# shanice-l/UNOPose

Hardware: AMD Instinct MI355X
Metric: (query,ref) pairs/sec forward (higher is better)
Workload: dtype bf16; 1 GPU; UNOPose.forward, batch 32 pairs/GPU, 2048 query pts, 5000->2048 reference pts, 196 coarse pts, 518x518 crops, DINOv2 ViT-B/14 reg4, random-init (trained-like) weights

## Files before the change

### include/unopose_hip.h

```cpp
#ifndef UNOPOSE_HIP_H
#define UNOPOSE_HIP_H

#include <stdint.h>

#ifdef __cplusplus
extern "C" {
#endif

#define UNOPOSE_OK 0
#define UNOPOSE_EINVAL 1
#define UNOPOSE_ELAUNCH 2
#define UNOPOSE_ENOMEM 3

typedef void *unopose_stream_t;

int unopose_abi_version(void);
const char *unopose_last_error(void);


int unopose_furthest_point_sampling(const float *xyz, int B, int N, int M,
                                    int32_t *idx, unopose_stream_t stream);

int unopose_gather_points(const float *points, const int32_t *idx, int B, int C,
                          int N, int M, float *out, unopose_stream_t stream);
// ... 41 lines not shown
                                const float *w, int M, int N, float thresh,
                                float eps, float *R, float *t,
                                unopose_stream_t stream);

int unopose_pe_image_bytes(void);
int unopose_pe_pack_weights(const float *w1, const float *b1, const float *w2, const float *b2,
                            const float *w3, const float *b3, void *image, unopose_stream_t stream);
int unopose_pe_group_mlp_max_packed(const float *xyz, int B, int N, float radius, int nsample,
                                    const void *image, float *out, unopose_stream_t stream);

int unopose_pe_group_mlp_max_packed_cand(const float *xyz, int B, int N, float radius, int nsample,
                                         const void *image, const int *cand_in, const int *cand_cnt_in,
                                         int cand_stride, int *cand_out, int *cand_cnt_out, float *out,
                                         unopose_stream_t stream);
int unopose_pe_group_mlp_max_packed_out(const float *xyz, int B, int N, float radius, int nsample, const void *image,
                                        const int *cand_in, const int *cand_cnt_in, int cand_stride, int *cand_out,
                                        int *cand_cnt_out, void *out, int out_ld, int out_split, unopose_stream_t stream);

int unopose_geo_embedding(const float *points, int B, int n, const void *wd_hi,
                          const void *wd_lo, const void *wa_hi, const void *wa_lo,
                          const float *bias_sum, const float *div_term,
                          float sigma_d, float factor_a, int reduce_mean, int split,
                          int out_bf16, int32_t *knn_ws, void *out,
                          unopose_stream_t stream);

int unopose_geo_embedding_table(const float *points, int B, int n, const float *tab_d, int rows_d, const float *tab_a, int rows_a,
                                const float *bias_sum, const float *w_d, const float *div_term, int hinv, int npoint, float sigma_d,
                                float factor_a, int reduce_mean, int out_bf16, int32_t *knn_ws, void *out,
                                unopose_stream_t stream);

// ... 197 lines not shown
```

### unopose_amd/_lib.py

```python
import ctypes
import os

import torch

_HERE = os.path.dirname(os.path.abspath(__file__))
SO_PATH = os.environ.get("UNOPOSE_LIB") or os.path.join(_HERE, "libunopose_hip.so")

_lib = None

_P = ctypes.c_void_p
_I = ctypes.c_int
_F = ctypes.c_float
_L = ctypes.c_long

SIGNATURES = {
    "unopose_furthest_point_sampling": [_P, _I, _I, _I, _P, _P],
    "unopose_gather_points": [_P, _P, _I, _I, _I, _I, _P, _P],
    "unopose_gather_points_grad": [_P, _P, _I, _I, _I, _I, _P, _P],
    "unopose_ball_query": [_P, _P, _I, _I, _I, _F, _I, _P, _P],
    "unopose_group_points": [_P, _P, _I, _I, _I, _I, _I, _P, _P],
    "unopose_group_points_grad": [_P, _P, _I, _I, _I, _I, _I, _P, _P],
    "unopose_three_nn": [_P, _P, _I, _I, _I, _P, _P, _P],
    "unopose_three_interpolate": [_P, _P, _P, _I, _I, _I, _I, _P, _P],
    "unopose_three_interpolate_grad": [_P, _P, _P, _I, _I, _I, _I, _P, _P],
# ... 66 lines not shown
    "unopose_overlap_scores": [_P, _I, _I, _I, _I, _I, _P, _P],
    "unopose_copy_rows": [_P, _L, _P, _L, _I, _I, _P],
    "unopose_nan_to_num_multi": [_P, _P, _I, _L, _F, _F, _F, _P],
    "unopose_rigid_rows_bf16": [_P, _I, _I, _P, _P, _P, _P],
    "unopose_token_sum_bf16": [_P, _I, _I, _I, _P, _P],
    "unopose_pose_score": [_P, _P, _I, _I, _F, _P, _P],
    "unopose_render_depth": [_P, _I, _P, _I, _P, _P, _I, _I, _I, _P, _P],
    "unopose_bmm_f32": [_P, ctypes.c_long, ctypes.c_long, ctypes.c_long, ctypes.c_long, _P, ctypes.c_long, ctypes.c_long, ctypes.c_long, ctypes.c_long, _P, _I, _I, _I, _I, _I, _F, _P],
    "unopose_split_bf16x2": [_P, ctypes.c_long, _I, _P, _P],
    "unopose_linear_f32x3": [_P, _P, _P, _P, _P, ctypes.c_long, _I, _I, _I, _P],
    "unopose_pe_image_bytes": [],
    "unopose_pe_pack_weights": [_P, _P, _P, _P, _P, _P, _P, _P],
    "unopose_pe_group_mlp_max_packed": [_P, _I, _I, _F, _I, _P, _P, _P],
    "unopose_pe_group_mlp_max_packed_cand": [_P, _I, _I, _F, _I, _P, _P, _P, _I, _P, _P, _P, _P],
    "unopose_pe_group_mlp_max_packed_out": [_P, _I, _I, _F, _I, _P, _P, _P, _I, _P, _P, _P, _I, _I, _P],
    "unopose_linear_f32x3_bf16": [_P, _P, _P, _P, _P, ctypes.c_long, _I, _I, _P],
    "unopose_pe_group_mlp_max": [_P, _I, _I, _F, _I, _P, _P, _P, _P, _P, _P, _I, _P, _P],
    "unopose_geo_embedding": [_P, _I, _I, _P, _P, _P, _P, _P, _P, _F, _F, _I, _I, _I, _P, _P, _P],
    "unopose_geo_embedding_train_workgroups": [_I, _I],
    "unopose_geo_embedding_train_forward": [_P, _I, _I, _P, _I, _P, _I, _P, _P, _P, _I, _F, _F, _I, _P, _P, _P, _P],
    "unopose_geo_embedding_train_backward": [_P, _P, _I, _I, _I, _I, _I, _F, _F, _I, _P, _P, _P, _P, _P, _P],
    "unopose_geo_embedding_table": [_P, _I, _I, _P, _I, _P, _I, _P, _P, _P, _I, _I, _F, _F, _I, _I, _P, _P, _P],
}


def lib():
    global _lib
    if _lib is None:
        if not os.path.exists(SO_PATH):
            raise RuntimeError(
# ... 70 lines not shown
```

### unopose_amd/csrc/pe.hip

```cpp
#include "common.h"
#include "jacobi3.h"

namespace unopose {

constexpr int PE_SCAN_STEPS = 4;

__device__ __forceinline__ int cd_row(int r, int h) { return (r & 3) + 8 * (r >> 2) + 4 * h; }

constexpr int PE_GDIM = 8, PE_GCELLS = PE_GDIM * PE_GDIM * PE_GDIM;
struct PeGrid {
  float ox, oy, oz, ihx, ihy, ihz;
  int nx, ny, nz;
  const u16 *start;
  const u16 *order;
  uint32_t *bits;
};
__device__ __forceinline__ int pe_cell(float v, float o, float ih, int n) { return max(0, min(n - 1, (int)((v - o) * ih))); }

template <typename NT>
__device__ __forceinline__ int pe_centre_frame(const float *sx, const float *sy, const float *sz, int N, int S,
                                               float radius, float r2, int lane, float cx, float cy, float cz,
                                               NT *nbr, Vec3 &xp, Vec3 &yp, Vec3 &zp, const int *cand = nullptr,
                                               int ncand = -1, const PeGrid *grid = nullptr) {
  int cnt = 0, first = 0;
// ... 279 lines not shown
    L->w2l[o][pe_kperm(c)] = f2bf(v - bf2f(h));
  }
  for (int e = tid; e < 128 * 64; e += 256) {
    const int o = e >> 6, c = e & 63;
    const float v = w3[e];
    const u16 h = f2bf(v);
    const int kp = pe_kperm(c) ^ ((o & 7) << 3);
    L->w3h[o][kp] = h;
    L->w3l[o][kp] = f2bf(v - bf2f(h));
  }
  if (tid < 32) L->b1[tid] = b1[tid];
  if (tid < 64) L->b2[tid] = b2[tid];
  if (tid < 128) L->b3[tid] = b3[tid];
}

constexpr int PE_NW = 4;
__global__ __launch_bounds__(PE_NW * 64, 8 / PE_NW) void pe_group_mlp_max_bf16x3_kernel(
    const float *__restrict__ xyz, int N, float radius, int S, int cpw, const uint4 *__restrict__ image,
    const int *__restrict__ cand_in, const int *__restrict__ cand_cnt_in, int cand_stride, int *__restrict__ cand_out,
    int *__restrict__ cand_cnt_out, float *__restrict__ out, int out_ld, int out_split, int use_grid) {
  extern __shared__ float4 smem4[];
  PeLdsB *L = reinterpret_cast<PeLdsB *>(smem4);
  float *sx = reinterpret_cast<float *>(L + 1);
  float *sy = sx + N, *sz = sy + N;
  float *stage_all = sz + N;
  u16 *nbr_all = reinterpret_cast<u16 *>(stage_all + PE_NW * 128);
  u16 *gstart = nbr_all + PE_NW * S;
  u16 *gorder = gstart + PE_GCELLS + 2;
  const int b = blockIdx.y, tid = threadIdx.x, lane = tid & 63, wave = tid >> 6;
  const int half = lane >> 5, col = lane & 31;
  u16 *nbr = nbr_all + wave * S;
  float *stage = stage_all + wave * 128;
  const float *P = xyz + (size_t)b * N * 3;

  for (int e = tid; e < N * 3; e += PE_NW * 64) {
    const float v = P[e];
    const int p = e / 3, comp = e - p * 3;
    (comp == 0 ? sx : comp == 1 ? sy : sz)[p] = v;
  }
  for (int e = tid; e < (int)(sizeof(PeLdsB) / 16); e += PE_NW * 64) smem4[e] = *reinterpret_cast<const float4 *>(image + e);
  __syncthreads();
  const float r2 = radius * radius;
  PeGrid grid;
  if (use_grid) {
    static_assert(PE_NW * 128 >= PE_GCELLS, "the cell counters borrow the staging area");
    uint32_t *cnt32 = reinterpret_cast<uint32_t *>(stage_all);
    float *red = reinterpret_cast<float *>(nbr_all);
    float lo[3] = {3e38f, 3e38f, 3e38f}, hi[3] = {-3e38f, -3e38f, -3e38f};
    for (int p = tid; p < N; p += PE_NW * 64) {
      lo[0] = fminf(lo[0], sx[p]), hi[0] = fmaxf(hi[0], sx[p]);
      lo[1] = fminf(lo[1], sy[p]), hi[1] = fmaxf(hi[1], sy[p]);
      lo[2] = fminf(lo[2], sz[p]), hi[2] = fmaxf(hi[2], sz[p]);
    }
#pragma unroll
    for (int a = 0; a < 3; ++a) {
      lo[a] = -wave_max_f32(-lo[a]);
      hi[a] = wave_max_f32(hi[a]);
      if (lane == 0) red[wave * 6 + a] = lo[a], red[wave * 6 + 3 + a] = hi[a];
    }
    for (int c = tid; c < PE_GCELLS; c += PE_NW * 64) cnt32[c] = 0u;
    __syncthreads();
    float org[3], ih[3];
    int nd[3];
#pragma unroll
    for (int a = 0; a < 3; ++a) {
      float l = red[a], h = red[3 + a];
      for (int w = 1; w < PE_NW; ++w) l = fminf(l, red[w * 6 + a]), h = fmaxf(h, red[w * 6 + 3 + a]);
      const float ext = h - l, h0 = radius * 1.001f;
      int n = (int)(ext / h0) + 1;
      float edge = h0;
      if (!(n <= PE_GDIM)) n = PE_GDIM, edge = fmaxf(h0, ext / (float)PE_GDIM * 1.001f);
      org[a] = __int_as_float(__builtin_amdgcn_readfirstlane(__float_as_int(l)));
      ih[a] = __int_as_float(__builtin_amdgcn_readfirstlane(__float_as_int(1.f / edge)));
      nd[a] = __builtin_amdgcn_readfirstlane(max(n, 1));
    }
    grid.ox = org[0], grid.oy = org[1], grid.oz = org[2], grid.ihx = ih[0], grid.ihy = ih[1], grid.ihz = ih[2];
    grid.nx = nd[0], grid.ny = nd[1], grid.nz = nd[2];
    grid.start = gstart, grid.order = gorder, grid.bits = reinterpret_cast<uint32_t *>(stage);
    auto cell_of = [&](int p) {
      return (pe_cell(sz[p], grid.oz, grid.ihz, grid.nz) * grid.ny + pe_cell(sy[p], grid.oy, grid.ihy, grid.ny)) * grid.nx +
             pe_cell(sx[p], grid.ox, grid.ihx, grid.nx);
    };
    for (int p = tid; p < N; p += PE_NW * 64) atomicAdd(&cnt32[cell_of(p)], 1u);
    __syncthreads();
    {
      constexpr int CPT = PE_GCELLS / (PE_NW * 64);
      static_assert(CPT * PE_NW * 64 == PE_GCELLS, "cells divide among the threads");
      uint32_t c[CPT], sum = 0;
#pragma unroll
      for (int e = 0; e < CPT; ++e) c[e] = cnt32[tid * CPT + e], sum += c[e];
      uint32_t incl = sum;
#pragma unroll
      for (int d = 1; d < 64; d <<= 1) {
        const uint32_t t = __shfl_up(incl, d);
        if (lane >= d) incl += t;
      }
      uint32_t *wtot = reinterpret_cast<uint32_t *>(red) + 32;
      if (lane == 63) wtot[wave] = incl;
      __syncthreads();
      uint32_t base = incl - sum;
      for (int w = 0; w < wave; ++w) base += wtot[w];
#pragma unroll
      for (int e = 0; e < CPT; ++e) {
        gstart[tid * CPT + e] = (u16)base;
        cnt32[tid * CPT + e] = base;
        base += c[e];
      }
      if (tid == PE_NW * 64 - 1) gstart[PE_GCELLS] = (u16)base;
    }
    __syncthreads();
    for (int p = tid; p < N; p += PE_NW * 64) gorder[atomicAdd(&cnt32[cell_of(p)], 1u)] = (u16)p;
    __syncthreads();
  }

  for (int ci = 0; ci < cpw; ++ci) {
    const int j = (blockIdx.x * PE_NW + wave) * cpw + ci;
    if (j >= N) break;
    const float cx = sx[j], cy = sy[j], cz = sz[j];
    Vec3 xp, yp, zp;
    const int *cand = nullptr;
    int ncand = -1;
    if (cand_in) {
      ncand = cand_cnt_in[(size_t)b * N + j];
      cand = cand_in + ((size_t)b * N + j) * cand_stride;
    }
    const int cnt = pe_centre_frame(sx, sy, sz, N, S, radius, r2, lane, cx, cy, cz, nbr, xp, yp, zp, cand, ncand, use_grid ? &grid : nullptr);
    if (cand_out) {
      int *co = cand_out + ((size_t)b * N + j) * S;
      for (int l = lane; l < S; l += 64) co[l] = nbr[l];
      if (lane == 0) cand_cnt_out[(size_t)b * N + j] = cnt <= S ? cnt : -1;
    }

    f32x16 rmax[4];
#pragma unroll
    for (int t = 0; t < 4; ++t)
#pragma unroll
      for (int r = 0; r < 16; ++r) rmax[t][r] = 0.f;
    const int S_eff = min(S, (max(min(cnt, S), 1) + 31) & ~31);
    for (int t0 = 0; t0 < S_eff; t0 += 32) {
      asm volatile("" ::: "memory");
      const int k = nbr[t0 + col];
      const float dx = sx[k] - cx, dy = sy[k] - cy, dz = sz[k] - cz;
      const Vec3 q = v3(dx / radius, dy / radius, dz / radius);
      float f[8] = {dx, dy, dz, dot(xp, q), dot(yp, q), dot(zp, q), 0.f, 0.f};
      if (half) {
#pragma unroll
        for (int e = 0; e < 8; ++e) f[e] = 0.f;
      }
      const bf16x8_hl x = split8_bf16(f);
      struct Grp {
        bf16x8_hl w[4];
        float4 b[4];
      } ga, gb;
      auto load_l1 = [&](Grp &g) {
        g.w[0].hi = *reinterpret_cast<const bf16x8 *>(&L->w1h[col][half * 8]);
        g.w[0].lo = *reinterpret_cast<const bf16x8 *>(&L->w1l[col][half * 8]);
#pragma unroll
        for (int q = 0; q < 4; ++q) g.b[q] = *reinterpret_cast<const float4 *>(&L->b1[8 * q + 4 * half]);
      };
      auto load_l2 = [&](Grp &g, int ot) {
#pragma unroll
        for (int ks = 0; ks < 2; ++ks) {
          g.w[ks].hi = *reinterpret_cast<const bf16x8 *>(&L->w2h[ot * 32 + col][ks * 16 + half * 8]);
          g.w[ks].lo = *reinterpret_cast<const bf16x8 *>(&L->w2l[ot * 32 + col][ks * 16 + half * 8]);
        }
#pragma unroll
        for (int q = 0; q < 4; ++q) g.b[q] = *reinterpret_cast<const float4 *>(&L->b2[ot * 32 + 8 * q + 4 * half]);
      };
      auto load_l3 = [&](Grp &g, int ot) {
        const int row = ot * 32 + col;
#pragma unroll
        for (int ks = 0; ks < 4; ++ks) {
          const int kp = (ks * 16 + half * 8) ^ ((row & 7) << 3);
          g.w[ks].hi = *reinterpret_cast<const bf16x8 *>(&L->w3h[row][kp]);
          g.w[ks].lo = *reinterpret_cast<const bf16x8 *>(&L->w3l[row][kp]);
        }
#pragma unroll
        for (int q = 0; q < 4; ++q) g.b[q] = *reinterpret_cast<const float4 *>(&L->b3[ot * 32 + 8 * q + 4 * half]);
      };
      auto init = [&](f32x16 &h, const Grp &g) {
#pragma unroll
        for (int q = 0; q < 4; ++q) {
          h[4 * q + 0] = g.b[q].x;
          h[4 * q + 1] = g.b[q].y;
          h[4 * q + 2] = g.b[q].z;
          h[4 * q + 3] = g.b[q].w;
        }
      };
      bf16x8_hl a1[2], a2[4];
      auto relu_split = [&](const f32x16 &h, bf16x8_hl *o) {
#pragma unroll
        for (int s2 = 0; s2 < 2; ++s2) {
          float v[8];
#pragma unroll
          for (int e = 0; e < 8; ++e) v[e] = fmaxf(h[s2 * 8 + e], 0.f);
          o[s2] = split8_bf16(v);
        }
      };
      load_l1(ga);
      load_l2(gb, 0);
      __builtin_amdgcn_sched_barrier(0);
      {
        f32x16 h1;
        init(h1, ga);
        h1 = mfma3_hh_hl_lh_32x32(ga.w[0], x, h1);
        load_l2(ga, 1);
        __builtin_amdgcn_sched_barrier(0);
        relu_split(h1, a1);
      }
      {
        f32x16 h2;
        init(h2, gb);
#pragma unroll
        for (int ks = 0; ks < 2; ++ks) h2 = mfma3_hh_hl_lh_32x32(gb.w[ks], a1[ks], h2);
        load_l3(gb, 0);
        __builtin_amdgcn_sched_barrier(0);
        relu_split(h2, a2);
        init(h2, ga);
#pragma unroll
        for (int ks = 0; ks < 2; ++ks) h2 = mfma3_hh_hl_lh_32x32(ga.w[ks], a1[ks], h2);
        load_l3(ga, 1);
        __builtin_amdgcn_sched_barrier(0);
        relu_split(h2, a2 + 2);
      }
#pragma unroll
      for (int ot = 0; ot < 4; ++ot) {
        Grp &g = (ot & 1) ? ga : gb;
        f32x16 h3;
        init(h3, g);
#pragma unroll
        for (int ks = 0; ks < 4; ++ks) h3 = mfma3_hh_hl_lh_32x32(g.w[ks], a2[ks], h3);
        if (ot + 2 < 4) {
          load_l3(g, ot + 2);
          __builtin_amdgcn_sched_barrier(0);
        }
#pragma unroll
        for (int r = 0; r < 16; ++r) rmax[ot][r] = fmaxf(rmax[ot][r], h3[r]);
      }
    }
#pragma unroll
    for (int t = 0; t < 4; ++t)
#pragma unroll
      for (int r = 0; r < 16; ++r) {
        float v = rmax[t][r];
        v = fmaxf(v, dpp_f32<0x111, 0xF>(v, 0.f));
        v = fmaxf(v, dpp_f32<0x112, 0xF>(v, 0.f));
        v = fmaxf(v, dpp_f32<0x114, 0xF>(v, 0.f));
        v = fmaxf(v, dpp_f32<0x118, 0xF>(v, 0.f));
        v = fmaxf(v, dpp_f32<0x142, 0xA>(v, 0.f));
        if (col == 31) stage[t * 32 + cd_row(r, half)] = v;
      }
    __builtin_amdgcn_fence(__ATOMIC_RELEASE, "wavefront");
    __builtin_amdgcn_wave_barrier();
    __builtin_amdgcn_fence(__ATOMIC_ACQUIRE, "wavefront");
    float *O = out + ((size_t)b * N + j) * out_ld;
    if (!out_split) {
      O[lane] = stage[lane];
      O[lane + 64] = stage[lane + 64];
    } else {
      uint32_t *O32 = reinterpret_cast<uint32_t *>(O);
#pragma unroll
      for (int q = 0; q < 2; ++q) {
        const int d = lane + 64 * q, blk = d >> 5, w = d & 31, k = blk * 32 + (w & 15) * 2;
        const float v0 = stage[k], v1 = stage[k + 1];
        const uint32_t h = cvt_pk_bf16_f32(v0, v1);
        O32[d] = (w & 16) ? cvt_pk_bf16_lo(v0, v1, h) : h;
      }
    }
    __builtin_amdgcn_wave_barrier();
  }
}

}

using namespace unopose;

extern "C" {

int unopose_pe_image_bytes(void) { return (int)sizeof(PeLdsB); }

int unopose_pe_pack_weights(const float *w1, const float *b1, const float *w2, const float *b2, const float *w3,
                            const float *b3, void *image, unopose_stream_t stream) {
  UNOPOSE_REQUIRE(w1 && b1 && w2 && b2 && w3 && b3 && image, "pe_pack_weights: null pointer");
  hipLaunchKernelGGL(pe_pack_weights_kernel, dim3(1), dim3(256), 0, (hipStream_t)stream, w1, b1, w2, b2, w3, b3,
// ... 2 lines not shown
}

int unopose_pe_group_mlp_max_packed(const float *xyz, int B, int N, float radius, int nsample, const void *image,
                                    float *out, unopose_stream_t stream) {
  return unopose_pe_group_mlp_max_packed_cand(xyz, B, N, radius, nsample, image, nullptr, nullptr, 0, nullptr, nullptr,
                                              out, stream);
}

int unopose_pe_group_mlp_max_packed_cand(const float *xyz, int B, int N, float radius, int nsample, const void *image,
                                         const int *cand_in, const int *cand_cnt_in, int cand_stride, int *cand_out,
                                         int *cand_cnt_out, float *out, unopose_stream_t stream) {
  return unopose_pe_group_mlp_max_packed_out(xyz, B, N, radius, nsample, image, cand_in, cand_cnt_in, cand_stride, cand_out,
                                             cand_cnt_out, out, 128, 0, stream);
}

int unopose_pe_group_mlp_max_packed_out(const float *xyz, int B, int N, float radius, int nsample, const void *image,
                                        const int *cand_in, const int *cand_cnt_in, int cand_stride, int *cand_out,
                                        int *cand_cnt_out, void *out, int out_ld, int out_split, unopose_stream_t stream) {
  UNOPOSE_REQUIRE(xyz && image && out, "pe_group_mlp_max_packed: null pointer");
  UNOPOSE_REQUIRE(out_ld >= 128 && (out_split == 0 || out_split == 1), "pe_group_mlp_max_packed: bad output stride / mode");
  UNOPOSE_REQUIRE((cand_in == nullptr) == (cand_cnt_in == nullptr) && (cand_out == nullptr) == (cand_cnt_out == nullptr) &&
                      (!cand_in || cand_stride >= 1),
                  "pe_group_mlp_max_packed: candidate list and its counts go together");
  UNOPOSE_REQUIRE(B >= 0 && N >= 1 && nsample >= 32 && nsample % 32 == 0 && B <= 65535,
                  "pe_group_mlp_max_packed: nsample must be a positive multiple of 32 (got %d)", nsample);
  if (B == 0) return UNOPOSE_OK;
  size_t lds = sizeof(PeLdsB) + ((size_t)3 * N + PE_NW * 128) * 4 + (size_t)PE_NW * nsample * 2;
  UNOPOSE_REQUIRE(N < 65536 && lds <= 160 * 1024, "pe_group_mlp_max_packed: N=%d nsample=%d exceed the LDS tile", N, nsample);
  const size_t grid_bytes = ((size_t)PE_GCELLS + 2 + (size_t)N) * 2;
  const int use_grid = radius > 0.f && N <= 4096 && N >= 256 && lds + grid_bytes <= 160 * 1024 && (lds + grid_bytes <= 80 * 1024 || lds > 80 * 1024);
  if (use_grid) lds += grid_bytes;
  lds = (lds + 15) & ~(size_t)15;
  static bool opt[64];
  if (lds_optin(opt, (const void *)pe_group_mlp_max_bf16x3_kernel, 160 * 1024, "pe_group_mlp_max_packed") != UNOPOSE_OK) return UNOPOSE_ELAUNCH;
  const long centres = (long)B * N;
  const int cpw = centres >= 65536 ? 16 : centres >= 32768 ? 8 : centres >= 8192 ? 4 : centres >= 2048 ? 2 : 1;
  dim3 grid(cdiv(N, PE_NW * cpw), B);
  hipLaunchKernelGGL(pe_group_mlp_max_bf16x3_kernel, grid, dim3(PE_NW * 64), lds, (hipStream_t)stream, xyz, N, radius, nsample,
                     cpw, (const uint4 *)image, cand_in, cand_cnt_in, cand_stride, cand_out, cand_cnt_out, (float *)out, out_ld, out_split, use_grid);
  return check_launch("pe_group_mlp_max_packed");
}

int unopose_pe_group_mlp_max(const float *xyz, int B, int N, float radius, int nsample, const float *w1,
                             const float *b1, const float *w2, const float *b2, const float *w3, const float *b3,
                             int bf16x3, float *out, unopose_stream_t stream) {
  UNOPOSE_REQUIRE(xyz && w1 && b1 && w2 && b2 && w3 && b3 && out, "pe_group_mlp_max: null pointer");
  UNOPOSE_REQUIRE(B >= 0 && N >= 1 && nsample >= 32 && nsample % 32 == 0 && B <= 65535,
                  "pe_group_mlp_max: nsample must be a positive multiple of 32 (got %d)", nsample);
  if (B == 0) return UNOPOSE_OK;
  const size_t lds = sizeof(PeLds) + ((size_t)3 * N + 4 * (size_t)nsample + 4 * 128) * 4;
  UNOPOSE_REQUIRE(lds <= 160 * 1024, "pe_group_mlp_max: N=%d nsample=%d exceed the LDS tile", N, nsample);
  static bool opt[64];
  if (lds_optin(opt, (const void *)pe_group_mlp_max_kernel, 160 * 1024, "pe_group_mlp_max") != UNOPOSE_OK) return UNOPOSE_ELAUNCH;
  const long centres = (long)B * N;
  const int cpw = centres >= 32768 ? 8 : centres >= 8192 ? 4 : centres >= 2048 ? 2 : 1;
// ... 10 lines not shown
```

Measured before the change: 1099 pairs/s.

## Split PE kernel into producer/consumer waves with LDS ring buffer

Restructures the point-embedding group+MLP+max kernel so four producer waves do the neighbour search and local frame while four consumer waves run the MFMA MLP. The two sides hand work through an LDS ring of neighbour lists and frames, using ticket counters and ready/freed flags. The point is to overlap the scalar-heavy ball query with the matrix-core MLP. Work per workgroup is now sized so the launch has about 512 workgroups. The old kernel is kept as a reference entry point, and the spin-wait sync adds deadlock and occupancy risk.

```diff
diff --git a/include/unopose_hip.h b/include/unopose_hip.h
--- a/include/unopose_hip.h
+++ b/include/unopose_hip.h
@@ -79,6 +79,9 @@
                                          int cand_stride, int *cand_out, int *cand_cnt_out, float *out,
                                          unopose_stream_t stream);
 int unopose_pe_group_mlp_max_packed_out(const float *xyz, int B, int N, float radius, int nsample, const void *image,
+                                        const int *cand_in, const int *cand_cnt_in, int cand_stride, int *cand_out,
+                                        int *cand_cnt_out, void *out, int out_ld, int out_split, unopose_stream_t stream);
+int unopose_pe_group_mlp_max_packed_ref(const float *xyz, int B, int N, float radius, int nsample, const void *image,
                                         const int *cand_in, const int *cand_cnt_in, int cand_stride, int *cand_out,
                                         int *cand_cnt_out, void *out, int out_ld, int out_split, unopose_stream_t stream);
 
diff --git a/unopose_amd/_lib.py b/unopose_amd/_lib.py
--- a/unopose_amd/_lib.py
+++ b/unopose_amd/_lib.py
@@ -104,6 +104,7 @@
     "unopose_pe_group_mlp_max_packed": [_P, _I, _I, _F, _I, _P, _P, _P],
     "unopose_pe_group_mlp_max_packed_cand": [_P, _I, _I, _F, _I, _P, _P, _P, _I, _P, _P, _P, _P],
     "unopose_pe_group_mlp_max_packed_out": [_P, _I, _I, _F, _I, _P, _P, _P, _I, _P, _P, _P, _I, _I, _P],
+    "unopose_pe_group_mlp_max_packed_ref": [_P, _I, _I, _F, _I, _P, _P, _P, _I, _P, _P, _P, _I, _I, _P],
     "unopose_linear_f32x3_bf16": [_P, _P, _P, _P, _P, ctypes.c_long, _I, _I, _P],
     "unopose_pe_group_mlp_max": [_P, _I, _I, _F, _I, _P, _P, _P, _P, _P, _P, _I, _P, _P],
     "unopose_geo_embedding": [_P, _I, _I, _P, _P, _P, _P, _P, _P, _F, _F, _I, _I, _I, _P, _P, _P],
diff --git a/unopose_amd/csrc/pe.hip b/unopose_amd/csrc/pe.hip
--- a/unopose_amd/csrc/pe.hip
+++ b/unopose_amd/csrc/pe.hip
@@ -317,9 +317,315 @@
   if (tid < 128) L->b3[tid] = b3[tid];
 }
 
-constexpr int PE_NW = 4;
-__global__ __launch_bounds__(PE_NW * 64, 8 / PE_NW) void pe_group_mlp_max_bf16x3_kernel(
+template <int NW>
+__device__ PeGrid pe_build_grid(const float *sx, const float *sy, const float *sz, int N, float radius, int tid, int lane, int wave,
+                                uint32_t *cnt32, float *red, u16 *gstart, u16 *gorder) {
+  PeGrid grid;
+  float lo[3] = {3e38f, 3e38f, 3e38f}, hi[3] = {-3e38f, -3e38f, -3e38f};
+  for (int p = tid; p < N; p += NW * 64) {
+    lo[0] = fminf(lo[0], sx[p]), hi[0] = fmaxf(hi[0], sx[p]);
+    lo[1] = fminf(lo[1], sy[p]), hi[1] = fmaxf(hi[1], sy[p]);
+    lo[2] = fminf(lo[2], sz[p]), hi[2] = fmaxf(hi[2], sz[p]);
+  }
+#pragma unroll
+  for (int a = 0; a < 3; ++a) {
+    lo[a] = -wave_max_f32(-lo[a]);
+    hi[a] = wave_max_f32(hi[a]);
+    if (lane == 0) red[wave * 6 + a] = lo[a], red[wave * 6 + 3 + a] = hi[a];
+  }
+  for (int c = tid; c < PE_GCELLS; c += NW * 64) cnt32[c] = 0u;
+  __syncthreads();
+  float org[3], ih[3];
+  int nd[3];
+#pragma unroll
+  for (int a = 0; a < 3; ++a) {
+    float l = red[a], h = red[3 + a];
+    for (int w = 1; w < NW; ++w) l = fminf(l, red[w * 6 + a]), h = fmaxf(h, red[w * 6 + 3 + a]);
+    const float ext = h - l, h0 = radius * 1.001f;
+    int n = (int)(ext / h0) + 1;
+    float edge = h0;
+    if (!(n <= PE_GDIM)) n = PE_GDIM, edge = fmaxf(h0, ext / (float)PE_GDIM * 1.001f);
+    org[a] = __int_as_float(__builtin_amdgcn_readfirstlane(__float_as_int(l)));
+    ih[a] = __int_as_float(__builtin_amdgcn_readfirstlane(__float_as_int(1.f / edge)));
+    nd[a] = __builtin_amdgcn_readfirstlane(max(n, 1));
+  }
+  grid.ox = org[0], grid.oy = org[1], grid.oz = org[2], grid.ihx = ih[0], grid.ihy = ih[1], grid.ihz = ih[2];
+  grid.nx = nd[0], grid.ny = nd[1], grid.nz = nd[2];
+  grid.start = gstart, grid.order = gorder, grid.bits = nullptr;
+  auto cell_of = [&](int p) {
+    return (pe_cell(sz[p], grid.oz, grid.ihz, grid.nz) * grid.ny + pe_cell(sy[p], grid.oy, grid.ihy, grid.ny)) * grid.nx +
+           pe_cell(sx[p], grid.ox, grid.ihx, grid.nx);
+  };
+  for (int p = tid; p < N; p += NW * 64) atomicAdd(&cnt32[cell_of(p)], 1u);
+  __syncthreads();
+  {
+    constexpr int CPT = PE_GCELLS / (NW * 64);
+    static_assert(CPT * NW * 64 == PE_GCELLS, "cells divide among the threads");
+    uint32_t c[CPT], sum = 0;
+#pragma unroll
+    for (int e = 0; e < CPT; ++e) c[e] = cnt32[tid * CPT + e], sum += c[e];
+    uint32_t incl = sum;
+#pragma unroll
+    for (int d = 1; d < 64; d <<= 1) {
+      const uint32_t t = __shfl_up(incl, d);
+      if (lane >= d) incl += t;
+    }
+    uint32_t *wtot = reinterpret_cast<uint32_t *>(red) + 6 * NW;
+    if (lane == 63) wtot[wave] = incl;
+    __syncthreads();
+    uint32_t base = incl - sum;
+    for (int w = 0; w < wave; ++w) base += wtot[w];
+#pragma unroll
+    for (int e = 0; e < CPT; ++e) {
+      gstart[tid * CPT + e] = (u16)base;
+      cnt32[tid * CPT + e] = base;
+      base += c[e];
+    }
+    if (tid == NW * 64 - 1) gstart[PE_GCELLS] = (u16)base;
+  }
+  __syncthreads();
+  for (int p = tid; p < N; p += NW * 64) gorder[atomicAdd(&cnt32[cell_of(p)], 1u)] = (u16)p;
+  __syncthreads();
+  return grid;
+}
+
+__device__ __forceinline__ void pe_mlp_tiles(const PeLdsB *L, const float *sx, const float *sy, const float *sz, const u16 *nbr,
+                                             int S_eff, float cx, float cy, float cz, float radius, Vec3 xp, Vec3 yp, Vec3 zp,
+                                             int half, int col, f32x16 (&rmax)[4]) {
+#pragma unroll
+  for (int t = 0; t < 4; ++t)
+#pragma unroll
+    for (int r = 0; r < 16; ++r) rmax[t][r] = 0.f;
+  for (int t0 = 0; t0 < S_eff; t0 += 32) {
+    asm volatile("" ::: "memory");
+    const int k = nbr[t0 + col];
+    const float dx = sx[k] - cx, dy = sy[k] - cy, dz = sz[k] - cz;
+    const Vec3 q = v3(dx / radius, dy / radius, dz / radius);
+    float f[8] = {dx, dy, dz, dot(xp, q), dot(yp, q), dot(zp, q), 0.f, 0.f};
+    if (half) {
+#pragma unroll
+      for (int e = 0; e < 8; ++e) f[e] = 0.f;
+    }
+    const bf16x8_hl x = split8_bf16(f);
+    struct Grp {
+      bf16x8_hl w[4];
+      float4 b[4];
+    } ga, gb;
+    auto load_l1 = [&](Grp &g) {
+      g.w[0].hi = *reinterpret_cast<const bf16x8 *>(&L->w1h[col][half * 8]);
+      g.w[0].lo = *reinterpret_cast<const bf16x8 *>(&L->w1l[col][half * 8]);
+#pragma unroll
+      for (int q = 0; q < 4; ++q) g.b[q] = *reinterpret_cast<const float4 *>(&L->b1[8 * q + 4 * half]);
+    };
+    auto load_l2 = [&](Grp &g, int ot) {
+#pragma unroll
+      for (int ks = 0; ks < 2; ++ks) {
+        g.w[ks].hi = *reinterpret_cast<const bf16x8 *>(&L->w2h[ot * 32 + col][ks * 16 + half * 8]);
+        g.w[ks].lo = *reinterpret_cast<const bf16x8 *>(&L->w2l[ot * 32 + col][ks * 16 + half * 8]);
+      }
+#pragma unroll
+      for (int q = 0; q < 4; ++q) g.b[q] = *reinterpret_cast<const float4 *>(&L->b2[ot * 32 + 8 * q + 4 * half]);
+    };
+    auto load_l3 = [&](Grp &g, int ot) {
+      const int row = ot * 32 + col;
+#pragma unroll
+      for (int ks = 0; ks < 4; ++ks) {
+        const int kp = (ks * 16 + half * 8) ^ ((row & 7) << 3);
+        g.w[ks].hi = *reinterpret_cast<const bf16x8 *>(&L->w3h[row][kp]);
+        g.w[ks].lo = *reinterpret_cast<const bf16x8 *>(&L->w3l[row][kp]);
+      }
+#pragma unroll
+      for (int q = 0; q < 4; ++q) g.b[q] = *reinterpret_cast<const float4 *>(&L->b3[ot * 32 + 8 * q + 4 * half]);
+    };
+    auto init = [&](f32x16 &h, const Grp &g) {
+#pragma unroll
+      for (int q = 0; q < 4; ++q) {
+        h[4 * q + 0] = g.b[q].x;
+        h[4 * q + 1] = g.b[q].y;
+        h[4 * q + 2] = g.b[q].z;
+        h[4 * q + 3] = g.b[q].w;
+      }
+    };
+    bf16x8_hl a1[2], a2[4];
+    auto relu_split = [&](const f32x16 &h, bf16x8_hl *o) {
+#pragma unroll
+      for (int s2 = 0; s2 < 2; ++s2) {
+        float v[8];
+#pragma unroll
+        for (int e = 0; e < 8; ++e) v[e] = fmaxf(h[s2 * 8 + e], 0.f);
+        o[s2] = split8_bf16(v);
+      }
+    };
+    load_l1(ga);
+    load_l2(gb, 0);
+    __builtin_amdgcn_sched_barrier(0);
+    {
+      f32x16 h1;
+      init(h1, ga);
+      h1 = mfma3_hh_hl_lh_32x32(ga.w[0], x, h1);
+      load_l2(ga, 1);
+      __builtin_amdgcn_sched_barrier(0);
+      relu_split(h1, a1);
+    }
+    {
+      f32x16 h2;
+      init(h2, gb);
+#pragma unroll
+      for (int ks = 0; ks < 2; ++ks) h2 = mfma3_hh_hl_lh_32x32(gb.w[ks], a1[ks], h2);
+      load_l3(gb, 0);
+      __builtin_amdgcn_sched_barrier(0);
+      relu_split(h2, a2);
+      init(h2, ga);
+#pragma unroll
+      for (int ks = 0; ks < 2; ++ks) h2 = mfma3_hh_hl_lh_32x32(ga.w[ks], a1[ks], h2);
+      load_l3(ga, 1);
+      __builtin_amdgcn_sched_barrier(0);
+      relu_split(h2, a2 + 2);
+    }
+#pragma unroll
+    for (int ot = 0; ot < 4; ++ot) {
+      Grp &g = (ot & 1) ? ga : gb;
+      f32x16 h3;
+      init(h3, g);
+#pragma unroll
+      for (int ks = 0; ks < 4; ++ks) h3 = mfma3_hh_hl_lh_32x32(g.w[ks], a2[ks], h3);
+      if (ot + 2 < 4) {
+        load_l3(g, ot + 2);
+        __builtin_amdgcn_sched_barrier(0);
+      }
+#pragma unroll
+      for (int r = 0; r < 16; ++r) rmax[ot][r] = fmaxf(rmax[ot][r], h3[r]);
+    }
+  }
+}
+
+__device__ __forceinline__ void pe_store_row(const f32x16 (&rmax)[4], float *stage, void *O, int out_split, int lane, int half,
+                                             int col) {
+#pragma unroll
+  for (int t = 0; t < 4; ++t)
+#pragma unroll
+    for (int r = 0; r < 16; ++r) {
+      float v = rmax[t][r];
+      v = fmaxf(v, dpp_f32<0x111, 0xF>(v, 0.f));
+      v = fmaxf(v, dpp_f32<0x112, 0xF>(v, 0.f));
+      v = fmaxf(v, dpp_f32<0x114, 0xF>(v, 0.f));
+      v = fmaxf(v, dpp_f32<0x118, 0xF>(v, 0.f));
+      v = fmaxf(v, dpp_f32<0x142, 0xA>(v, 0.f));
+      if (col == 31) stage[t * 32 + cd_row(r, half)] = v;
+    }
+  __builtin_amdgcn_fence(__ATOMIC_RELEASE, "wavefront");
+  __builtin_amdgcn_wave_barrier();
+  __builtin_amdgcn_fence(__ATOMIC_ACQUIRE, "wavefront");
+  if (!out_split) {
+    float *Of = reinterpret_cast<float *>(O);
+    Of[lane] = stage[lane];
+    Of[lane + 64] = stage[lane + 64];
+  } else {
+    uint32_t *O32 = reinterpret_cast<uint32_t *>(O);
+#pragma unroll
+    for (int q = 0; q < 2; ++q) {
+      const int d = lane + 64 * q, blk = d >> 5, w = d & 31, k = blk * 32 + (w & 15) * 2;
+      const float v0 = stage[k], v1 = stage[k + 1];
+      const uint32_t h = cvt_pk_bf16_f32(v0, v1);
+      O32[d] = (w & 16) ? cvt_pk_bf16_lo(v0, v1, h) : h;
+    }
+  }
+  __builtin_amdgcn_wave_barrier();
+}
+
+__device__ __forceinline__ const int *pe_cand_in(const int *cand_in, const int *cand_cnt_in, int cand_stride, int N, int b, int j,
+                                                 int &ncand) {
+  ncand = -1;
+  if (!cand_in) return nullptr;
+  ncand = cand_cnt_in[(size_t)b * N + j];
+  return cand_in + ((size_t)b * N + j) * cand_stride;
+}
+__device__ __forceinline__ void pe_cand_out(int *cand_out, int *cand_cnt_out, int N, int S, int b, int j, const u16 *nbr, int cnt,
+                                            int lane) {
+  if (!cand_out) return;
+  int *co = cand_out + ((size_t)b * N + j) * S;
+  for (int l = lane; l < S; l += 64) co[l] = nbr[l];
+  if (lane == 0) cand_cnt_out[(size_t)b * N + j] = cnt <= S ? cnt : -1;
+}
+
+__device__ __forceinline__ int pe_tiles_needed(int cnt, int S) { return min(S, (max(min(cnt, S), 1) + 31) & ~31); }
+
+constexpr int PE_REF_NW = 4;
+__global__ __launch_bounds__(PE_REF_NW * 64, 8 / PE_REF_NW) void pe_group_mlp_max_bf16x3_ref_kernel(
     const float *__restrict__ xyz, int N, float radius, int S, int cpw, const uint4 *__restrict__ image,
+    const int *__restrict__ cand_in, const int *__restrict__ cand_cnt_in, int cand_stride, int *__restrict__ cand_out,
+    int *__restrict__ cand_cnt_out, float *__restrict__ out, int out_ld, int out_split, int use_grid) {
+  constexpr int NW = PE_REF_NW;
+  extern __shared__ float4 smem4[];
+  PeLdsB *L = reinterpret_cast<PeLdsB *>(smem4);
+  float *sx = reinterpret_cast<float *>(L + 1);
+  float *sy = sx + N, *sz = sy + N;
+  float *stage_all = sz + N;
+  u16 *nbr_all = reinterpret_cast<u16 *>(stage_all + NW * 128);
+  u16 *gstart = nbr_all + NW * S;
+  u16 *gorder = gstart + PE_GCELLS + 2;
+  const int b = blockIdx.y, tid = threadIdx.x, lane = tid & 63, wave = tid >> 6;
+  const int half = lane >> 5, col = lane & 31;
+  u16 *nbr = nbr_all + wave * S;
+  float *stage = stage_all + wave * 128;
+  const float *P = xyz + (size_t)b * N * 3;
+
+  for (int e = tid; e < N * 3; e += NW * 64) {
+    const float v = P[e];
+    const int p = e / 3, comp = e - p * 3;
+    (comp == 0 ? sx : comp == 1 ? sy : sz)[p] = v;
+  }
+  for (int e = tid; e < (int)(sizeof(PeLdsB) / 16); e += NW * 64) smem4[e] = *reinterpret_cast<const float4 *>(image + e);
+  __syncthreads();
+  const float r2 = radius * radius;
+  PeGrid grid;
+  if (use_grid) {
+    static_assert(NW * 128 >= PE_GCELLS, "the cell counters borrow the staging area");
+    grid = pe_build_grid<NW>(sx, sy, sz, N, radius, tid, lane, wave, reinterpret_cast<uint32_t *>(stage_all),
+                             reinterpret_cast<float *>(nbr_all), gstart, gorder);
+    grid.bits = reinterpret_cast<uint32_t *>(stage);
+  }
+
+  for (int ci = 0; ci < cpw; ++ci) {
+    const int j = (blockIdx.x * NW + wave) * cpw + ci;
+    if (j >= N) break;
+    const float cx = sx[j], cy = sy[j], cz = sz[j];
+    Vec3 xp, yp, zp;
+    int ncand;
+    const int *cand = pe_cand_in(cand_in, cand_cnt_in, cand_stride, N, b, j, ncand);
+    const int cnt = pe_centre_frame(sx, sy, sz, N, S, radius, r2, lane, cx, cy, cz, nbr, xp, yp, zp, cand, ncand, use_grid ? &grid : nullptr);
+    pe_cand_out(cand_out, cand_cnt_out, N, S, b, j, nbr, cnt, lane);
+    f32x16 rmax[4];
+    pe_mlp_tiles(L, sx, sy, sz, nbr, pe_tiles_needed(cnt, S), cx, cy, cz, radius, xp, yp, zp, half, col, rmax);
+    pe_store_row(rmax, stage, out + ((size_t)b * N + j) * out_ld, out_split, lane, half, col);
+  }
+}
+
+constexpr int PE_NC = 4, PE_NP = 4, PE_NWP = PE_NC + PE_NP;
+constexpr int PE_RING = 8;
+constexpr int PE_FRAME = 12;
+constexpr int PE_SPIN_MAX = 1 << 22;
+constexpr long PE_WG_TARGET = 512;
+
+__device__ __forceinline__ bool pe_wait_ge(uint32_t *flag, uint32_t v) {
+  for (int n = 0; n < PE_SPIN_MAX; ++n) {
+    if ((uint32_t)__builtin_amdgcn_readfirstlane(__hip_atomic_load(flag, __ATOMIC_ACQUIRE, __HIP_MEMORY_SCOPE_WORKGROUP)) >= v) return true;
+    __builtin_amdgcn_s_sleep(1);
+  }
+  return false;
+}
+__device__ __forceinline__ void pe_post(uint32_t *flag, uint32_t v, int lane) {
+  __builtin_amdgcn_fence(__ATOMIC_RELEASE, "workgroup");
+  if (lane == 0) __hip_atomic_store(flag, v, __ATOMIC_RELAXED, __HIP_MEMORY_SCOPE_WORKGROUP);
+}
+__device__ __forceinline__ int pe_ticket(uint32_t *ctr, int lane) {
+  uint32_t k = 0;
+  if (lane == 0) k = atomicAdd(ctr, 1u);
+  return __builtin_amdgcn_readlane((int)k, 0);
+}
+
+__global__ __launch_bounds__(PE_NWP * 64, 2) void pe_group_mlp_max_bf16x3_kernel(
+    const float *__restrict__ xyz, int N, float radius, int S, int cpg, const uint4 *__restrict__ image,
     const int *__restrict__ cand_in, const int *__restrict__ cand_cnt_in, int cand_stride, int *__restrict__ cand_out,
     int *__restrict__ cand_cnt_out, float *__restrict__ out, int out_ld, int out_split, int use_grid) {
   extern __shared__ float4 smem4[];
@@ -327,250 +633,72 @@
   float *sx = reinterpret_cast<float *>(L + 1);
   float *sy = sx + N, *sz = sy + N;
   float *stage_all = sz + N;
-  u16 *nbr_all = reinterpret_cast<u16 *>(stage_all + PE_NW * 128);
-  u16 *gstart = nbr_all + PE_NW * S;
+  uint32_t *bits_all = reinterpret_cast<uint32_t *>(stage_all + PE_NC * 128);
+  float *frames = reinterpret_cast<float *>(bits_all + PE_NP * 128);
+  uint32_t *ctrl = reinterpret_cast<uint32_t *>(frames + PE_RING * PE_FRAME);
+  uint32_t *ready = ctrl + 2, *freed = ready + PE_RING;
+  u16 *lists = reinterpret_cast<u16 *>(freed + PE_RING);
+  u16 *gstart = lists + PE_RING * S;
   u16 *gorder = gstart + PE_GCELLS + 2;
   const int b = blockIdx.y, tid = threadIdx.x, lane = tid & 63, wave = tid >> 6;
-  const int half = lane >> 5, col = lane & 31;
-  u16 *nbr = nbr_all + wave * S;
-  float *stage = stage_all + wave * 128;
+  const int j0 = blockIdx.x * cpg, nj = min(cpg, N - j0);
   const float *P = xyz + (size_t)b * N * 3;
 
-  for (int e = tid; e < N * 3; e += PE_NW * 64) {
+  for (int e = tid; e < N * 3; e += PE_NWP * 64) {
     const float v = P[e];
     const int p = e / 3, comp = e - p * 3;
     (comp == 0 ? sx : comp == 1 ? sy : sz)[p] = v;
   }
-  for (int e = tid; e < (int)(sizeof(PeLdsB) / 16); e += PE_NW * 64) smem4[e] = *reinterpret_cast<const float4 *>(image + e);
+  for (int e = tid; e < (int)(sizeof(PeLdsB) / 16); e += PE_NWP * 64) smem4[e] = *reinterpret_cast<const float4 *>(image + e);
+  if (tid < 2 + 2 * PE_RING) ctrl[tid] = 0u;
   __syncthreads();
-  const float r2 = radius * radius;
   PeGrid grid;
   if (use_grid) {
-    static_assert(PE_NW * 128 >= PE_GCELLS, "the cell counters borrow the staging area");
-    uint32_t *cnt32 = reinterpret_cast<uint32_t *>(stage_all);
-    float *red = reinterpret_cast<float *>(nbr_all);
-    float lo[3] = {3e38f, 3e38f, 3e38f}, hi[3] = {-3e38f, -3e38f, -3e38f};
-    for (int p = tid; p < N; p += PE_NW * 64) {
-      lo[0] = fminf(lo[0], sx[p]), hi[0] = fmaxf(hi[0], sx[p]);
-      lo[1] = fminf(lo[1], sy[p]), hi[1] = fmaxf(hi[1], sy[p]);
-      lo[2] = fminf(lo[2], sz[p]), hi[2] = fmaxf(hi[2], sz[p]);
-    }
-#pragma unroll
-    for (int a = 0; a < 3; ++a) {
-      lo[a] = -wave_max_f32(-lo[a]);
-      hi[a] = wave_max_f32(hi[a]);
-      if (lane == 0) red[wave * 6 + a] = lo[a], red[wave * 6 + 3 + a] = hi[a];
-    }
-    for (int c = tid; c < PE_GCELLS; c += PE_NW * 64) cnt32[c] = 0u;
-    __syncthreads();
-    float org[3], ih[3];
-    int nd[3];
-#pragma unroll
-    for (int a = 0; a < 3; ++a) {
-      float l = red[a], h = red[3 + a];
-      for (int w = 1; w < PE_NW; ++w) l = fminf(l, red[w * 6 + a]), h = fmaxf(h, red[w * 6 + 3 + a]);
-      const float ext = h - l, h0 = radius * 1.001f;
-      int n = (int)(ext / h0) + 1;
-      float edge = h0;
-      if (!(n <= PE_GDIM)) n = PE_GDIM, edge = fmaxf(h0, ext / (float)PE_GDIM * 1.001f);
-      org[a] = __int_as_float(__builtin_amdgcn_readfirstlane(__float_as_int(l)));
-      ih[a] = __int_as_float(__builtin_amdgcn_readfirstlane(__float_as_int(1.f / edge)));
-      nd[a] = __builtin_amdgcn_readfirstlane(max(n, 1));
-    }
-    grid.ox = org[0], grid.oy = org[1], grid.oz = org[2], grid.ihx = ih[0], grid.ihy = ih[1], grid.ihz = ih[2];
-    grid.nx = nd[0], grid.ny = nd[1], grid.nz = nd[2];
-    grid.start = gstart, grid.order = gorder, grid.bits = reinterpret_cast<uint32_t *>(stage);
-    auto cell_of = [&](int p) {
-      return (pe_cell(sz[p], grid.oz, grid.ihz, grid.nz) * grid.ny + pe_cell(sy[p], grid.oy, grid.ihy, grid.ny)) * grid.nx +
-             pe_cell(sx[p], grid.ox, grid.ihx, grid.nx);
-    };
-    for (int p = tid; p < N; p += PE_NW * 64) atomicAdd(&cnt32[cell_of(p)], 1u);
-    __syncthreads();
-    {
-      constexpr int CPT = PE_GCELLS / (PE_NW * 64);
-      static_assert(CPT * PE_NW * 64 == PE_GCELLS, "cells divide among the threads");
-      uint32_t c[CPT], sum = 0;
-#pragma unroll
-      for (int e = 0; e < CPT; ++e) c[e] = cnt32[tid * CPT + e], sum += c[e];
-      uint32_t incl = sum;
-#pragma unroll
-      for (int d = 1; d < 64; d <<= 1) {
-        const uint32_t t = __shfl_up(incl, d);
-        if (lane >= d) incl += t;
-      }
-      uint32_t *wtot = reinterpret_cast<uint32_t *>(red) + 32;
-      if (lane == 63) wtot[wave] = incl;
-      __syncthreads();
-      uint32_t base = incl - sum;
-      for (int w = 0; w < wave; ++w) base += wtot[w];
-#pragma unroll
-      for (int e = 0; e < CPT; ++e) {
-        gstart[tid * CPT + e] = (u16)base;
-        cnt32[tid * CPT + e] = base;
-        base += c[e];
-      }
-      if (tid == PE_NW * 64 - 1) gstart[PE_GCELLS] = (u16)base;
-    }
-    __syncthreads();
-    for (int p = tid; p < N; p += PE_NW * 64) gorder[atomicAdd(&cnt32[cell_of(p)], 1u)] = (u16)p;
-    __syncthreads();
-  }
-
-  for (int ci = 0; ci < cpw; ++ci) {
-    const int j = (blockIdx.x * PE_NW + wave) * cpw + ci;
-    if (j >= N) break;
-    const float cx = sx[j], cy = sy[j], cz = sz[j];
-    Vec3 xp, yp, zp;
-    const int *cand = nullptr;
-    int ncand = -1;
-    if (cand_in) {
-      ncand = cand_cnt_in[(size_t)b * N + j];
-      cand = cand_in + ((size_t)b * N + j) * cand_stride;
-    }
-    const int cnt = pe_centre_frame(sx, sy, sz, N, S, radius, r2, lane, cx, cy, cz, nbr, xp, yp, zp, cand, ncand, use_grid ? &grid : nullptr);
-    if (cand_out) {
-      int *co = cand_out + ((size_t)b * N + j) * S;
-      for (int l = lane; l < S; l += 64) co[l] = nbr[l];
-      if (lane == 0) cand_cnt_out[(size_t)b * N + j] = cnt <= S ? cnt : -1;
-    }
-
-    f32x16 rmax[4];
-#pragma unroll
-    for (int t = 0; t < 4; ++t)
-#pragma unroll
-      for (int r = 0; r < 16; ++r) rmax[t][r] = 0.f;
-    const int S_eff = min(S, (max(min(cnt, S), 1) + 31) & ~31);
-    for (int t0 = 0; t0 < S_eff; t0 += 32) {
-      asm volatile("" ::: "memory");
-      const int k = nbr[t0 + col];
-      const float dx = sx[k] - cx, dy = sy[k] - cy, dz = sz[k] - cz;
-      const Vec3 q = v3(dx / radius, dy / radius, dz / radius);
-      float f[8] = {dx, dy, dz, dot(xp, q), dot(yp, q), dot(zp, q), 0.f, 0.f};
-      if (half) {
-#pragma unroll
-        for (int e = 0; e < 8; ++e) f[e] = 0.f;
-      }
-      const bf16x8_hl x = split8_bf16(f);
-      struct Grp {
-        bf16x8_hl w[4];
-        float4 b[4];
-      } ga, gb;
-      auto load_l1 = [&](Grp &g) {
-        g.w[0].hi = *reinterpret_cast<const bf16x8 *>(&L->w1h[col][half * 8]);
-        g.w[0].lo = *reinterpret_cast<const bf16x8 *>(&L->w1l[col][half * 8]);
-#pragma unroll
-        for (int q = 0; q < 4; ++q) g.b[q] = *reinterpret_cast<const float4 *>(&L->b1[8 * q + 4 * half]);
-      };
-      auto load_l2 = [&](Grp &g, int ot) {
-#pragma unroll
-        for (int ks = 0; ks < 2; ++ks) {
-          g.w[ks].hi = *reinterpret_cast<const bf16x8 *>(&L->w2h[ot * 32 + col][ks * 16 + half * 8]);
-          g.w[ks].lo = *reinterpret_cast<const bf16x8 *>(&L->w2l[ot * 32 + col][ks * 16 + half * 8]);
-        }
-#pragma unroll
-        for (int q = 0; q < 4; ++q) g.b[q] = *reinterpret_cast<const float4 *>(&L->b2[ot * 32 + 8 * q + 4 * half]);
-      };
-      auto load_l3 = [&](Grp &g, int ot) {
-        const int row = ot * 32 + col;
-#pragma unroll
-        for (int ks = 0; ks < 4; ++ks) {
-          const int kp = (ks * 16 + half * 8) ^ ((row & 7) << 3);
-          g.w[ks].hi = *reinterpret_cast<const bf16x8 *>(&L->w3h[row][kp]);
-          g.w[ks].lo = *reinterpret_cast<const bf16x8 *>(&L->w3l[row][kp]);
-        }
-#pragma unroll
-        for (int q = 0; q < 4; ++q) g.b[q] = *reinterpret_cast<const float4 *>(&L->b3[ot * 32 + 8 * q + 4 * half]);
-      };
-      auto init = [&](f32x16 &h, const Grp &g) {
-#pragma unroll
-        for (int q = 0; q < 4; ++q) {
-          h[4 * q + 0] = g.b[q].x;
-          h[4 * q + 1] = g.b[q].y;
-          h[4 * q + 2] = g.b[q].z;
-          h[4 * q + 3] = g.b[q].w;
-        }
-      };
-      bf16x8_hl a1[2], a2[4];
-      auto relu_split = [&](const f32x16 &h, bf16x8_hl *o) {
-#pragma unroll
-        for (int s2 = 0; s2 < 2; ++s2) {
-          float v[8];
-#pragma unroll
-          for (int e = 0; e < 8; ++e) v[e] = fmaxf(h[s2 * 8 + e], 0.f);
-          o[s2] = split8_bf16(v);
-        }
-      };
-      load_l1(ga);
-      load_l2(gb, 0);
-      __builtin_amdgcn_sched_barrier(0);
-      {
-        f32x16 h1;
-        init(h1, ga);
-        h1 = mfma3_hh_hl_lh_32x32(ga.w[0], x, h1);
-        load_l2(ga, 1);
-        __builtin_amdgcn_sched_barrier(0);
-        relu_split(h1, a1);
-      }
-      {
-        f32x16 h2;
-        init(h2, gb);
-#pragma unroll
-        for (int ks = 0; ks < 2; ++ks) h2 = mfma3_hh_hl_lh_32x32(gb.w[ks], a1[ks], h2);
-        load_l3(gb, 0);
-        __builtin_amdgcn_sched_barrier(0);
-        relu_split(h2, a2);
-        init(h2, ga);
-#pragma unroll
-        for (int ks = 0; ks < 2; ++ks) h2 = mfma3_hh_hl_lh_32x32(ga.w[ks], a1[ks], h2);
-        load_l3(ga, 1);
-        __builtin_amdgcn_sched_barrier(0);
-        relu_split(h2, a2 + 2);
-      }
-#pragma unroll
-      for (int ot = 0; ot < 4; ++ot) {
-        Grp &g = (ot & 1) ? ga : gb;
-        f32x16 h3;
-        init(h3, g);
-#pragma unroll
-        for (int ks = 0; ks < 4; ++ks) h3 = mfma3_hh_hl_lh_32x32(g.w[ks], a2[ks], h3);
-        if (ot + 2 < 4) {
-          load_l3(g, ot + 2);
-          __builtin_amdgcn_sched_barrier(0);
-        }
-#pragma unroll
-        for (int r = 0; r < 16; ++r) rmax[ot][r] = fmaxf(rmax[ot][r], h3[r]);
-      }
-    }
-#pragma unroll
-    for (int t = 0; t < 4; ++t)
-#pragma unroll
-      for (int r = 0; r < 16; ++r) {
-        float v = rmax[t][r];
-        v = fmaxf(v, dpp_f32<0x111, 0xF>(v, 0.f));
-        v = fmaxf(v, dpp_f32<0x112, 0xF>(v, 0.f));
-        v = fmaxf(v, dpp_f32<0x114, 0xF>(v, 0.f));
-        v = fmaxf(v, dpp_f32<0x118, 0xF>(v, 0.f));
-        v = fmaxf(v, dpp_f32<0x142, 0xA>(v, 0.f));
-        if (col == 31) stage[t * 32 + cd_row(r, half)] = v;
-      }
-    __builtin_amdgcn_fence(__ATOMIC_RELEASE, "wavefront");
-    __builtin_amdgcn_wave_barrier();
-    __builtin_amdgcn_fence(__ATOMIC_ACQUIRE, "wavefront");
-    float *O = out + ((size_t)b * N + j) * out_ld;
-    if (!out_split) {
-      O[lane] = stage[lane];
-      O[lane + 64] = stage[lane + 64];
-    } else {
-      uint32_t *O32 = reinterpret_cast<uint32_t *>(O);
-#pragma unroll
-      for (int q = 0; q < 2; ++q) {
-        const int d = lane + 64 * q, blk = d >> 5, w = d & 31, k = blk * 32 + (w & 15) * 2;
-        const float v0 = stage[k], v1 = stage[k + 1];
-        const uint32_t h = cvt_pk_bf16_f32(v0, v1);
-        O32[d] = (w & 16) ? cvt_pk_bf16_lo(v0, v1, h) : h;
-      }
-    }
-    __builtin_amdgcn_wave_barrier();
+    static_assert((PE_NC + PE_NP) * 128 >= PE_GCELLS && PE_RING * 32 * 2 >= 7 * PE_NWP * 4, "the grid build borrows the staging area, the bit maps and the lists");
+    grid = pe_build_grid<PE_NWP>(sx, sy, sz, N, radius, tid, lane, wave, reinterpret_cast<uint32_t *>(stage_all),
+                                 reinterpret_cast<float *>(lists), gstart, gorder);
+  }
+  if (wave >= PE_NC) {
+    grid.bits = bits_all + (wave - PE_NC) * 128;
+    const float r2 = radius * radius;
+    for (;;) {
+      const int k = pe_ticket(&ctrl[0], lane);
+      if (k >= nj) break;
+      const int s = k % PE_RING;
+      if (!pe_wait_ge(&freed[s], (uint32_t)(k / PE_RING))) return;
+      const int j = j0 + k;
+      const float cx = sx[j], cy = sy[j], cz = sz[j];
+      u16 *nbr = lists + s * S;
+      Vec3 xp, yp, zp;
+      int ncand;
+      const int *cand = pe_cand_in(cand_in, cand_cnt_in, cand_stride, N, b, j, ncand);
+      const int cnt = pe_centre_frame(sx, sy, sz, N, S, radius, r2, lane, cx, cy, cz, nbr, xp, yp, zp, cand, ncand, use_grid ? &grid : nullptr);
+      pe_cand_out(cand_out, cand_cnt_out, N, S, b, j, nbr, cnt, lane);
+      if (lane == 0) {
+        float *f = frames + s * PE_FRAME;
+        f[0] = xp.x, f[1] = xp.y, f[2] = xp.z, f[3] = yp.x, f[4] = yp.y, f[5] = yp.z, f[6] = zp.x, f[7] = zp.y, f[8] = zp.z;
+        f[9] = __int_as_float(cnt);
+      }
+      pe_post(&ready[s], (uint32_t)(k / PE_RING) + 1u, lane);
+    }
+  } else {
+    const int half = lane >> 5, col = lane & 31;
+    float *stage = stage_all + wave * 128;
+    for (;;) {
+      const int k = pe_ticket(&ctrl[1], lane);
+      if (k >= nj) break;
+      const int s = k % PE_RING;
+      if (!pe_wait_ge(&ready[s], (uint32_t)(k / PE_RING) + 1u)) return;
+      const int j = j0 + k;
+      const float cx = sx[j], cy = sy[j], cz = sz[j];
+      const float *f = frames + s * PE_FRAME;
+      const Vec3 xp = v3(f[0], f[1], f[2]), yp = v3(f[3], f[4], f[5]), zp = v3(f[6], f[7], f[8]);
+      const int cnt = __float_as_int(f[9]);
+      f32x16 rmax[4];
+      pe_mlp_tiles(L, sx, sy, sz, lists + s * S, pe_tiles_needed(cnt, S), cx, cy, cz, radius, xp, yp, zp, half, col, rmax);
+      pe_post(&freed[s], (uint32_t)(k / PE_RING) + 1u, lane);
+      pe_store_row(rmax, stage, out + ((size_t)b * N + j) * out_ld, out_split, lane, half, col);
+    }
   }
 }
 
@@ -603,9 +731,9 @@
                                              cand_cnt_out, out, 128, 0, stream);
 }
 
-int unopose_pe_group_mlp_max_packed_out(const float *xyz, int B, int N, float radius, int nsample, const void *image,
-                                        const int *cand_in, const int *cand_cnt_in, int cand_stride, int *cand_out,
-                                        int *cand_cnt_out, void *out, int out_ld, int out_split, unopose_stream_t stream) {
+static int pe_packed_launch(bool ref, const float *xyz, int B, int N, float radius, int nsample, const void *image, const int *cand_in,
+                            const int *cand_cnt_in, int cand_stride, int *cand_out, int *cand_cnt_out, void *out, int out_ld,
+                            int out_split, unopose_stream_t stream) {
   UNOPOSE_REQUIRE(xyz && image && out, "pe_group_mlp_max_packed: null pointer");
   UNOPOSE_REQUIRE(out_ld >= 128 && (out_split == 0 || out_split == 1), "pe_group_mlp_max_packed: bad output stride / mode");
   UNOPOSE_REQUIRE((cand_in == nullptr) == (cand_cnt_in == nullptr) && (cand_out == nullptr) == (cand_cnt_out == nullptr) &&
@@ -614,20 +742,49 @@
   UNOPOSE_REQUIRE(B >= 0 && N >= 1 && nsample >= 32 && nsample % 32 == 0 && B <= 65535,
                   "pe_group_mlp_max_packed: nsample must be a positive multiple of 32 (got %d)", nsample);
   if (B == 0) return UNOPOSE_OK;
-  size_t lds = sizeof(PeLdsB) + ((size_t)3 * N + PE_NW * 128) * 4 + (size_t)PE_NW * nsample * 2;
+  const size_t grid_bytes = ((size_t)PE_GCELLS + 2 + (size_t)N) * 2;
+  const long centres = (long)B * N;
+  if (ref) {
+    size_t lds = sizeof(PeLdsB) + ((size_t)3 * N + PE_REF_NW * 128) * 4 + (size_t)PE_REF_NW * nsample * 2;
+    UNOPOSE_REQUIRE(N < 65536 && lds <= 160 * 1024, "pe_group_mlp_max_packed: N=%d nsample=%d exceed the LDS tile", N, nsample);
+    const int use_grid = radius > 0.f && N <= 4096 && N >= 256 && lds + grid_bytes <= 160 * 1024 && (lds + grid_bytes <= 80 * 1024 || lds > 80 * 1024);
+    if (use_grid) lds += grid_bytes;
+    lds = (lds + 15) & ~(size_t)15;
+    static bool opt[64];
+    if (lds_optin(opt, (const void *)pe_group_mlp_max_bf16x3_ref_kernel, 160 * 1024, "pe_group_mlp_max_packed_ref") != UNOPOSE_OK) return UNOPOSE_ELAUNCH;
+    const int cpw = centres >= 65536 ? 16 : centres >= 32768 ? 8 : centres >= 8192 ? 4 : centres >= 2048 ? 2 : 1;
+    hipLaunchKernelGGL(pe_group_mlp_max_bf16x3_ref_kernel, dim3(cdiv(N, PE_REF_NW * cpw), B), dim3(PE_REF_NW * 64), lds, (hipStream_t)stream,
+                       xyz, N, radius, nsample, cpw, (const uint4 *)image, cand_in, cand_cnt_in, cand_stride, cand_out, cand_cnt_out,
+                       (float *)out, out_ld, out_split, use_grid);
+    return check_launch("pe_group_mlp_max_packed_ref");
+  }
+  size_t lds = sizeof(PeLdsB) + ((size_t)3 * N + (PE_NC + PE_NP) * 128 + PE_RING * PE_FRAME + 2 + 2 * PE_RING) * 4 +
+               (size_t)PE_RING * nsample * 2;
   UNOPOSE_REQUIRE(N < 65536 && lds <= 160 * 1024, "pe_group_mlp_max_packed: N=%d nsample=%d exceed the LDS tile", N, nsample);
-  const size_t grid_bytes = ((size_t)PE_GCELLS + 2 + (size_t)N) * 2;
-  const int use_grid = radius > 0.f && N <= 4096 && N >= 256 && lds + grid_bytes <= 160 * 1024 && (lds + grid_bytes <= 80 * 1024 || lds > 80 * 1024);
+  const int use_grid = radius > 0.f && N <= 4096 && N >= 256 && lds + grid_bytes <= 160 * 1024;
   if (use_grid) lds += grid_bytes;
   lds = (lds + 15) & ~(size_t)15;
   static bool opt[64];
   if (lds_optin(opt, (const void *)pe_group_mlp_max_bf16x3_kernel, 160 * 1024, "pe_group_mlp_max_packed") != UNOPOSE_OK) return UNOPOSE_ELAUNCH;
-  const long centres = (long)B * N;
-  const int cpw = centres >= 65536 ? 16 : centres >= 32768 ? 8 : centres >= 8192 ? 4 : centres >= 2048 ? 2 : 1;
-  dim3 grid(cdiv(N, PE_NW * cpw), B);
-  hipLaunchKernelGGL(pe_group_mlp_max_bf16x3_kernel, grid, dim3(PE_NW * 64), lds, (hipStream_t)stream, xyz, N, radius, nsample,
-                     cpw, (const uint4 *)image, cand_in, cand_cnt_in, cand_stride, cand_out, cand_cnt_out, (float *)out, out_ld, out_split, use_grid);
+  const int cpg = (int)min((long)N, max((long)(2 * PE_NC), (long)cdiv(centres, PE_WG_TARGET)));
+  hipLaunchKernelGGL(pe_group_mlp_max_bf16x3_kernel, dim3(cdiv(N, cpg), B), dim3(PE_NWP * 64), lds, (hipStream_t)stream, xyz, N, radius,
+                     nsample, cpg, (const uint4 *)image, cand_in, cand_cnt_in, cand_stride, cand_out, cand_cnt_out, (float *)out, out_ld,
+                     out_split, use_grid);
   return check_launch("pe_group_mlp_max_packed");
+}
+
+int unopose_pe_group_mlp_max_packed_out(const float *xyz, int B, int N, float radius, int nsample, const void *image,
+                                        const int *cand_in, const int *cand_cnt_in, int cand_stride, int *cand_out,
+                                        int *cand_cnt_out, void *out, int out_ld, int out_split, unopose_stream_t stream) {
+  return pe_packed_launch(false, xyz, B, N, radius, nsample, image, cand_in, cand_cnt_in, cand_stride, cand_out, cand_cnt_out, out,
+                          out_ld, out_split, stream);
+}
+
+int unopose_pe_group_mlp_max_packed_ref(const float *xyz, int B, int N, float radius, int nsample, const void *image,
+                                        const int *cand_in, const int *cand_cnt_in, int cand_stride, int *cand_out,
+                                        int *cand_cnt_out, void *out, int out_ld, int out_split, unopose_stream_t stream) {
+  return pe_packed_launch(true, xyz, B, N, radius, nsample, image, cand_in, cand_cnt_in, cand_stride, cand_out, cand_cnt_out, out,
+                          out_ld, out_split, stream);
 }
 
 int unopose_pe_group_mlp_max(const float *xyz, int B, int N, float radius, int nsample, const float *w1,
```

Measured after the change: 1105 pairs/s (median of 6 runs). About the same (+0.5%).
